# zahmedy/PyTorch-Distributed-Data-Parallel-DDP-Trainer

Hardware: AMD Instinct MI355X
Metric: images/sec MNIST SimpleCNN DDP at 1/2/4/8 MI355X; DDP scaling efficiency (higher is better)
Workload: dtype bf16; 1 GPU; model=SimpleCNN (520,586 params), global_batch=32, per_rank_batch=32, image=1x28x28, parallelism=dp1, engine=fused hipGraph, graph_steps=7, graph_head=0, fuse_level=3, level3=True, params_finite=True, bucket_allreduce=none, params_identical_across_ranks=True, ranks_seen=1, force_allreduce=False, inlaunch_allreduce=False

## Files before the change

### csrc/bindings.cpp

```cpp
#include <torch/extension.h>
#include <c10/hip/HIPStream.h>

#include <optional>

#include "kernels/conv_infer.h"
#include "kernels/launchers.h"
#include "runtime/runtime.h"

namespace py = pybind11;
using at::Tensor;
using namespace ddp_amd;

extern "C" const char ddp_amd_source_hash_str[];

namespace {

hipStream_t cur_stream() { return c10::hip::getCurrentHIPStream().stream(); }

void check_cuda(const Tensor& t, const char* name) {
  TORCH_CHECK(t.is_cuda(), name, " must be a GPU tensor");
  TORCH_CHECK(t.is_contiguous(), name, " must be contiguous");
}
void check(const Tensor& t, const char* name, at::ScalarType st) {
  check_cuda(t, name);
// ... 1292 lines not shown
             c.wgrad_rows = cfgd["wgrad_rows"].cast<int>();
             c.world = cfgd["world"].cast<int>(); c.rank = cfgd["rank"].cast<int>();
             c.lr = cfgd["lr"].cast<float>(); c.momentum = cfgd["momentum"].cast<float>();
             c.dampening = cfgd["dampening"].cast<float>();
             c.weight_decay = cfgd["weight_decay"].cast<float>();
             c.nesterov = cfgd["nesterov"].cast<bool>(); c.maximize = cfgd["maximize"].cast<bool>();
             c.force_allreduce = cfgd.contains("force_allreduce") ? cfgd["force_allreduce"].cast<bool>() : false;
             c.fuse_level = cfgd.contains("fuse_level") ? cfgd["fuse_level"].cast<int>() : 0;
             c.fuse_opt = cfgd.contains("fuse_opt") ? (int)cfgd["fuse_opt"].cast<bool>() : 1;
             c.store_a1 = cfgd.contains("store_a1") ? cfgd["store_a1"].cast<int>() : 0;
             c.f32 = cfgd.contains("f32") ? (int)cfgd["f32"].cast<bool>() : 0;
             c.fuse_reduce = cfgd.contains("fuse_reduce") ? cfgd["fuse_reduce"].cast<int>() : 1;
             c.wgrad_split = cfgd.contains("wgrad_split") ? cfgd["wgrad_split"].cast<int>() : 1;
             c.l3_fc_role = cfgd.contains("l3_fc_role") ? cfgd["l3_fc_role"].cast<int>() : 1;
             c.dist_mode = cfgd.contains("dist_mode") ? cfgd["dist_mode"].cast<int>() : 3;
             TORCH_CHECK(c.dist_mode >= 0 && c.dist_mode <= 4, "engine: dist_mode must be 0..4");
             TORCH_CHECK(c.l3_fc_role == 0 || c.l3_fc_role == 1, "engine: l3_fc_role must be 0 or 1");
             TORCH_CHECK(c.wgrad_split == 1 || c.wgrad_split == 2, "engine: wgrad_split must be 1 or 2");
             const int es = c.f32 ? 4 : 2;
             TORCH_CHECK(c.store_a1 >= 0 && c.store_a1 <= 2, "engine: store_a1 must be 0, 1 or 2");
             TORCH_CHECK(c.fuse_level == 0 || c.fuse_level == 1 || c.fuse_level == 3,
                         "engine: fuse_level must be 0, 1 or 3 (level 2 was removed in round 4)");
             TORCH_CHECK(conv3x3_fwd_lds(c.W, c.C1, c.pxt_fwd, c.fuse_level > 0, es) <= 160 * 1024 &&
                             conv3x3_wgrad_lds(c.W, c.C1, c.C2, c.wgrad_rows, c.fuse_level > 0, es) <= 160 * 1024 &&
                             conv3x3_dgrad_lds(c.W, c.C2, c.pxt_dgrad, true, es) <= 160 * 1024,
                         "engine: LDS budget exceeded for this tiling");
             auto T = [&](const char* k) { return t[k].cast<Tensor>(); };
             auto need = [&](const char* k, at::ScalarType st, long n) {
               Tensor x = T(k);
               check(x, k, st);
// ... 70 lines not shown
      .def("capture", &SimpleCNNEngine::capture)
      .def("replay", &SimpleCNNEngine::replay)
      .def("destroy_graph", &SimpleCNNEngine::destroy_graph)
      .def("synchronize", &SimpleCNNEngine::synchronize, py::call_guard<py::gil_scoped_release>())
      .def_property_readonly("last_fused_reduce", &SimpleCNNEngine::last_fused_reduce)
      .def_property_readonly("last_level3", &SimpleCNNEngine::last_level3)
      .def_property_readonly("last_fc_role", &SimpleCNNEngine::last_fc_role)
      .def_property_readonly("last_xar", &SimpleCNNEngine::last_xar)
      .def_property_readonly("last_pair", &SimpleCNNEngine::last_pair)
      .def_property_readonly("last_head", &SimpleCNNEngine::last_head)
      .def_property_readonly("graph_heads", &SimpleCNNEngine::graph_heads)
      .def("overlap_active", &SimpleCNNEngine::overlap_active)
      .def("level3_active", &SimpleCNNEngine::level3_active, py::arg("batch"))
      .def_property_readonly("sync_error", &SimpleCNNEngine::sync_error)
      .def("set_momentum_started", &SimpleCNNEngine::set_momentum_started)
      .def("set_xgmi", &SimpleCNNEngine::set_xgmi, py::arg("xgmi"), py::arg("channels"))
      .def_property_readonly("num_buckets", &SimpleCNNEngine::num_buckets)
      .def("bucket_stage", &SimpleCNNEngine::bucket_stage)
      .def_property_readonly("graph_steps", &SimpleCNNEngine::graph_steps)
      .def_property_readonly("stream", [](SimpleCNNEngine& e) { return (uint64_t)e.stream(); });
}
```

### csrc/kernels/conv3x3_fwd_body.inc.h

```cpp
  using P = Prec<T>;
  constexpr bool F32 = sizeof(T) == 4;
  static_assert(!DZ || (NOF == 10 && A1X), "level-3 dZ2 needs the fc epilogue and the conv1 recompute");
  static_assert(!MRG || (DZ && !F32), "the merged forward is the bf16 level-3 forward");
  constexpr int CE = P::CE;
  DDP_STAMP(STAMP_K_CONV_FWD, 0);
  DDP_GEOM_OVERRIDE();
  typedef __attribute__((address_space(1))) unsigned long long gran_t;
  constexpr int DZ_SW = (OCC == 2 || F32) ? XENT_MAX_BLK / 2 : XENT_MAX_BLK;
  unsigned dz_epoch = 1u;
  if constexpr (DZ) {
    const unsigned g = *dzo.gen + 1u;
    dz_epoch = g ? g : 1u;
  }
  constexpr int CH = 16 * NW * PXT, NT = NW * 64;
  const int lane = threadIdx.x & 63, wave = threadIdx.x >> 6;
  const int HW = H * W;
  const long Ptot = (long)B * HW;
  const int co0 = by * 64;
  const int KW = 9 * Cin, WS = KW + P::PAD, XS = Cin + P::PAD;
  const int XR = CH + 2 * W + 2;
  T* sW = reinterpret_cast<T*>(smem);
  T* sX = sW + 64 * WS;
  const long P0 = (long)bx * CH;
  const long Pbase = P0 - W - 1;

  const int wc = KW / CE;
// ... 9 lines not shown
  if (A1X) cg = conv1_group_load(c1.w, c1.b, wave & 3);
  stage2<(64 / NW) * (F32 ? 2 : 1), NT>(64 * wc,
             [&](int i) { const int r = i / wc, c = (i - r * wc) * CE; return ld16(Wt + (long)(co0 + r) * KW + c); },
             [&](int i, bf16x8 v) { const int r = i / wc, c = (i - r * wc) * CE; st16(sW + r * WS + c, v); },
             A1X ? 0 : XR * xc,
             [&](int i) {
               const int r = i / xc, c = (i - r * xc) * CE;
               const long Pq = Pbase + r;
               return (Pq >= 0 && Pq < Ptot) ? ld16(X + Pq * Cin + c) : zero8();
             },
             [&](int i, bf16x8 v) { const int r = i / xc, c = (i - r * xc) * CE; st16(sX + r * XS + c, v); });
  }
  if (A1X) {
    float* sxx = reinterpret_cast<float*>(sX + XR * XS);
    const int NXX = XR + 2 * W + 2;
    const int base = bi_base = c1.bi.base();
    for (int r = threadIdx.x; r < NXX; r += NT) {
      const long Pq = Pbase - W - 1 + r;
      float v = 0.f;
      if (Pq >= 0 && Pq < Ptot) {
        const int n = (int)(Pq / HW), rm = (int)(Pq - (long)n * HW);
        const int row = c1.bi.row(n, base);
        const unsigned char u = c1.x[(long)row * HW + rm];
        v = (float)u / 255.0f;
        if (c1.xb_out && Pq >= P0 && Pq < P0 + CH) {
          c1.xb_out[Pq] = u;
          if (rm == 0) c1.yb_out[n] = c1.labels[row];
        }
      }
      sxx[r] = v;
    }
    if constexpr (MRG) {
      DDP_STAMP(STAMP_K_HEAD, 4);
      wait_count<MRG_SLEEP>(mg.conv_done, mg.nblk1, mg.err, MRG_ERR);
      DDP_STAMP(STAMP_K_HEAD, 5);
      cg = conv1_group_load_sc1(c1.w, c1.b, wave & 3);
      const __amdgpu_buffer_rsrc_t rw =
          __builtin_amdgcn_make_buffer_rsrc(const_cast<T*>(Wt), (short)0, 0x7fffffff, 0x00020000);
      stage2<64 / NW, NT>(64 * wc,
          [&](int i) { const int r = i / wc, c = (i - r * wc) * CE; return ld16_sc1(rw, (int)(((co0 + r) * KW + c) * sizeof(T))); },
          [&](int i, bf16x8 v) { const int r = i / wc, c = (i - r * wc) * CE; st16(sW + r * WS + c, v); },
          0, [&](int) { return zero8(); }, [&](int, bf16x8) {});
// ... 245 lines not shown
          const int co = co0 + 16 * t + 4 * (lane >> 4);
          if (!valid[pt]) continue;
          if constexpr (F32) st_wt(reinterpret_cast<float4*>(Y + Pp[pt] * Cout + co), a2q[pt][t]);
          else st_wt(reinterpret_cast<uint2*>(Y + Pp[pt] * Cout + co), a2pk[pt][t]);
        }
    };
    DDP_STAMP(STAMP_K_FWD_DZ, 0);
    store_a2();
    if (wave == 0) {
      const int slot = lane >= NOF ? 1 : 0, o = lane - slot * NOF;
      const bool act = lane < 2 * NOF && slot < nimg;
      int label = 0;
      float fcb = 0.f;
      if (lane < 2 * NOF) {
        const int im = img0 + slot;
        if (im < B) label = c1.labels[c1.bi.row(im, bi_base)];
        fcb = MRG ? __hip_atomic_load(dzo.fc_bias + o, __ATOMIC_RELAXED, __HIP_MEMORY_SCOPE_AGENT) : dzo.fc_bias[o];
      }
      const int im = img0 + (act ? slot : 0);
      const int nblk = (im * HWi + HWi - 1) / CH - im * HWi / CH + 1;
      const gran_t* gr = (const gran_t*)dzo.gran;
      const unsigned long long t0 = __builtin_amdgcn_s_memrealtime();
      bool dead = false;
      float a = 0.f;
      DDP_STAMP(STAMP_K_FWD_DZ, 1);
      auto sweep = [&](auto j0c) {
        constexpr int J0 = decltype(j0c)::value;
        unsigned long long g[DZ_SW];
#pragma unroll
        for (int k = 0; k < DZ_SW; ++k) g[k] = 0;
        const bool none = J0 > 0 && !__any(act && nblk > J0);
// ... 86 lines not shown
```

### csrc/kernels/fc_bwd_body.h

```cpp
#pragma once
#include "kernels/common.h"
#include "kernels/launchers.h"

namespace ddp_amd {

constexpr int FCB_RB = 8;

template <int CPL>
struct ColF {
  float v[CPL];
};
template <int CPL>
__device__ __forceinline__ ColF<CPL> ldc(const bf16_t* p) {
  ColF<CPL> r;
  if constexpr (CPL == 2) {
    const unsigned u = *reinterpret_cast<const unsigned*>(p);
    r.v[0] = __builtin_bit_cast(float, u << 16);
    r.v[1] = __builtin_bit_cast(float, u & 0xffff0000u);
  } else {
    const uint2 u = *reinterpret_cast<const uint2*>(p);
    r.v[0] = __builtin_bit_cast(float, u.x << 16);
    r.v[1] = __builtin_bit_cast(float, u.x & 0xffff0000u);
    r.v[2] = __builtin_bit_cast(float, u.y << 16);
    r.v[3] = __builtin_bit_cast(float, u.y & 0xffff0000u);
// ... 55 lines not shown
    }
  }
  if ((XENT || ex.loss_rows) && ex.loss_out) {
    const float* lr = XENT ? s_loss : ex.loss_rows;
    const int at = ex.step_ctr ? *ex.step_ctr : 0;
    float acc = 0.f;
    for (int b0 = 0; b0 < B; b0 += 64) {
      const float v = b0 + lane < B ? lr[b0 + lane] : 0.f;
      const int nb = B - b0 < 64 ? B - b0 : 64;
      for (int k = 0; k < nb; ++k)
        acc += __builtin_bit_cast(float, __builtin_amdgcn_readlane(__builtin_bit_cast(int, v), k));
    }
    if (lane == 63) {
      ex.loss_out[at] = acc / (float)B;
      if (last && ex.step_inc) *ex.step_inc = at + 1;
    }
  }
  if (last || !ex.last_ctr) {
    if (ex.zero_i32)
      for (int i = lane; i < ex.n_zero; i += 64) ex.zero_i32[(long)i * ex.zero_stride] = 0;
    if (ex.gen_inc && lane == 0) {
      const unsigned g = *ex.gen_inc + 1u;
      *ex.gen_inc = g == 0xffffffffu ? 0u : g;
    }
  }
}

constexpr int FCDW_LD = 12;
template <int MAXB, typename T>
__device__ __forceinline__ void fc_dw_wave_chunk(const float* s_dl, const T* __restrict__ X,
// ... 273 lines not shown
```

### csrc/kernels/launchers.h

```cpp
#pragma once
#include <hip/hip_runtime.h>
#include <stdint.h>

#include "kernels/types.h"

namespace ddp_amd {

void stamps_set(void* buf);

void conv1_fwd(const void* x, bool x_is_u8, BatchIdx bi, const float* w, const float* b, bf16_t* y,
               int B, int H, int W, int Cout, hipStream_t s);
void conv1_fwd(const void* x, bool x_is_u8, BatchIdx bi, const float* w, const float* b, float* y,
               int B, int H, int W, int Cout, hipStream_t s);
int conv1_wgrad_blocks(int B, int H, int W, int chunk);
void conv1_wgrad(const void* x, bool x_is_u8, BatchIdx bi, const bf16_t* dy, const bf16_t* yact,
                 float* slab, int B, int H, int W, int Cout, int chunk, hipStream_t s);
void conv1_wgrad(const void* x, bool x_is_u8, BatchIdx bi, const float* dy, const float* yact,
                 float* slab, int B, int H, int W, int Cout, int chunk, hipStream_t s);

constexpr int FWD_DZ_CNT_STRIDE = 64;
struct FwdDz {
  bf16_t* dz2 = nullptr;
  float* dz2_f32 = nullptr;
  unsigned long long* gran = nullptr;
// ... 146 lines not shown
  const int* labels32 = nullptr;
  BatchIdx bi{};
  float gscale = 1.f;
  SgdArgs sgd{};
  float* p_w = nullptr;
  float* m_w = nullptr;
  bf16_t* sh_plain = nullptr;
  bf16_t* sh_frag = nullptr;
  float* sh_frag32 = nullptr;
  int frag_HW = 0, frag_C = 0;
  int sys_store = 0;
  int* last_ctr = nullptr;
  float* p_b = nullptr;
  float* m_b = nullptr;
  int* step_inc = nullptr;
  unsigned* gen_inc = nullptr;
  int* zero_i32 = nullptr;
  int n_zero = 0, zero_stride = 1;
  int last_n = 0;
};
struct BwdFc {
  const void* a2 = nullptr;
  const float* dl = nullptr;
  float* dW = nullptr;
  float scale = 1.f;
  long K = 0;
  int nconv = 0, fc0 = 0, nfc = 0;
  FcBwdExtras ex{};
};
size_t fc_bwd_lds(int B, int NO, bool xent, long npart = 0);
void noop(int blocks, int* sink, hipStream_t s);
void fc_bwd(const float* dL, const bf16_t* X, const bf16_t* Wf, bf16_t* dX, float* dW, float scale,
            int B, long K, int NO, bool mask, hipStream_t s, const FcBwdExtras& ex = FcBwdExtras());
void fc_bwd(const float* dL, const float* X, const float* Wf, float* dX, float* dW, float scale,
            int B, long K, int NO, bool mask, hipStream_t s, const FcBwdExtras& ex = FcBwdExtras());

void xent(const float* part, int G, const float* bias, int C, int B, const long long* labels64,
          const int* labels32, BatchIdx bi, float* logits_out, float* dlogits, float* loss_out,
          float* dbias, float gscale, float dbias_scale, hipStream_t s);

bool xent_wave_rows(const float* logits, int C, int B, const long long* labels, float* dlogits,
                    float* loss_out, float gscale, hipStream_t s);

void xent_rows(const float* part, int HW, int CH, const float* bias, int NO, int B,
               const int* labels32, BatchIdx bi, float* dlogits, float* loss_rows, float gscale,
               hipStream_t s);

enum { SHADOW_BF16 = 1, SHADOW_BF16_TAPT = 2, SHADOW_BF16_FCFRAG = 3, SHADOW_BF16_PAD4 = 4,
       SHADOW_F32_TAPT = 5, SHADOW_F32_FCFRAG = 6 };
constexpr int MAX_SHADOWS = 4;
// ... 119 lines not shown
```

### csrc/kernels/types.h

```cpp
#pragma once
#include <hip/hip_runtime.h>
#include <stdint.h>

namespace ddp_amd {

typedef unsigned short bf16_t;

struct BatchIdx {
  const int* idx;
  const int* step_ctr;
  int batch_stride;
  int offset;
  int n_idx = 0x7fffffff;
  int n_rows = 0x7fffffff;
  __device__ __forceinline__ int base() const {
    return step_ctr ? (*step_ctr) * batch_stride : offset;
  }
  __device__ __forceinline__ int row(int b, int base_) const {
    if (!idx) {
      const int r = base_ + b;
      return r < 0 ? 0 : (r >= n_rows ? n_rows - 1 : r);
    }
    int i = base_ + b;
    i = i < 0 ? 0 : (i >= n_idx ? n_idx - 1 : i);
    int r = idx[i];
    return r < 0 ? 0 : (r >= n_rows ? n_rows - 1 : r);
  }
};

struct C1Src {
  const unsigned char* x = nullptr;
  BatchIdx bi{};
  const float* w = nullptr;
  const float* b = nullptr;
  unsigned char* xb_out = nullptr;
  int* yb_out = nullptr;
  const int* labels = nullptr;
  bf16_t* a1_out = nullptr;
  int* zero_i32 = nullptr;
  int zero_per_block = 0;
  int zero_total = 0x7fffffff;
};

struct SgdArgs {
  float lr, momentum, dampening, weight_decay;
  int nesterov, maximize, first_step, update;
};

struct SchedState {
  int t, ticket;
  float lr_used;
};
// ... 22 lines not shown
```

### csrc/runtime/engine.cpp

```cpp
#include <algorithm>
#include <cstdio>
#include <cstdlib>
#include <cstring>
#include <type_traits>

#include "runtime/runtime.h"

namespace ddp_amd {

SimpleCNNEngine::SimpleCNNEngine(const EngineConfig& cfg, const EngineBuffers& buf,
                                 std::shared_ptr<Comm> comm, std::vector<EngineBucket> buckets)
    : cfg_(cfg), b_(buf), comm_(std::move(comm)), buckets_(std::move(buckets)) {
  if (cfg_.C1 != 32) throw std::runtime_error("engine: fused conv1 wgrad needs C1 == 32");
  if (cfg_.C2 % 64 != 0) throw std::runtime_error("engine: C2 must be a multiple of 64");
  if ((cfg_.H * cfg_.W) % 16 != 0) throw std::runtime_error("engine: H*W must be a multiple of 16");
  if (cfg_.NO != 10) throw std::runtime_error("engine: the fused fc epilogue is built for 10 classes");
  if (cfg_.f32 && (cfg_.fuse_level < 1 || cfg_.store_a1 != 0))
    throw std::runtime_error("engine: fp32 mode needs fuse_level >= 1 (level 1 or 3) and store_a1 0");
  if (cfg_.f32 && !(b_.a2_f32 && b_.dz2_f32 && b_.w2t_f32 && b_.wfc_frag32))
    throw std::runtime_error("engine: fp32 mode needs the a2 / dz2 / w2t / wfc_frag32 fp32 buffers");
  const long conv0 = std::min(std::min(b_.off_w2, b_.off_b2), std::min(b_.off_w1, b_.off_b1));
  const long fc_hi = std::max(b_.off_wfc + (long)cfg_.NO * cfg_.H * cfg_.W * cfg_.C2, b_.off_bfc + cfg_.NO);
  if (fc_hi > conv0) throw std::runtime_error("engine: fc gradients must precede the conv gradients");
  long prev_end = 0;
// ... 13 lines not shown
  l3_fits_.assign(cfg_.max_batch + 1, -1);
  if (b_.sync_err) {
    DDP_HIP_CHECK(hipHostMalloc(reinterpret_cast<void**>(&err_host_), sizeof(int),
                                hipHostMallocCoherent | hipHostMallocMapped));
    *err_host_ = 0;
    int* dev = nullptr;
    DDP_HIP_CHECK(hipHostGetDevicePointer(reinterpret_cast<void**>(&dev), err_host_, 0));
    b_.sync_err = dev;
  }
  if (cfg_.fuse_level >= 3 && b_.sync_flags && b_.sync_err) {
    const size_t ng = 2 * (size_t)cfg_.NO * (size_t)conv3x3_dgrad_blocks(cfg_.max_batch, cfg_.H, cfg_.W, 1);
    DDP_HIP_CHECK(hipMalloc(reinterpret_cast<void**>(&gran_), ng * sizeof(unsigned long long)));
    DDP_HIP_CHECK(hipMalloc(reinterpret_cast<void**>(&gen_), 256));
    DDP_HIP_CHECK(hipMemset(gran_, 0, ng * sizeof(unsigned long long)));
    DDP_HIP_CHECK(hipMemset(gen_, 0, 256));
    DDP_HIP_CHECK(hipStreamSynchronize(nullptr));
  }
}

SimpleCNNEngine::~SimpleCNNEngine() {
  if (process_exiting()) return;
  if (cs_) hipStreamSynchronize(cs_);
  destroy_graph();
  for (hipEvent_t e : {e_b0_, e_b1_, e_d0_, e_d1_, e_fwd_, e_fc_}) hipEventDestroy(e);
  for (XarArgs& e : xar_cache_) hipFree(const_cast<XgmiArgs*>(e.dev));
  if (err_host_) hipHostFree(err_host_);
  if (gran_) hipFree(gran_);
  if (gen_) hipFree(gen_);
}

void SimpleCNNEngine::destroy_graph() {
  if (graph_exec_) hipGraphExecDestroy(graph_exec_);
  if (graph_) hipGraphDestroy(graph_);
  graph_exec_ = nullptr;
  graph_ = nullptr;
  graph_steps_ = 0;
}

void SimpleCNNEngine::synchronize() {
  DDP_HIP_CHECK(hipStreamSynchronize(cs_));
  if (const int e = sync_error()) {
    throw std::runtime_error(std::string("engine: an in-launch hand-off wait timed out (") +
                             (e == RED_ERR ? "fused slab reduction" : e == XAR_ERR ? "in-launch all-reduce"
// ... 69 lines not shown
  if constexpr (std::is_same<T, float>::value)
    return {b.params + b.off_w2, b.w2t_f32, b.a2_f32, b.dz2_f32, b.wfc_frag32, b.params + b.off_wfc, nullptr, sh};
  else
    return {b.w2_bf16, b.w2t_bf16, b.a2, b.dz2, b.wfc_frag, b.wfc_bf16, b.a1, sh};
}

}

void SimpleCNNEngine::launch_step(int B, int stride, bool first_momentum_step, unsigned parts) {
  if (cfg_.f32)
    launch_step_t<float>(B, stride, first_momentum_step, parts);
  else
    launch_step_t<bf16_t>(B, stride, first_momentum_step, parts);
}

C1Src SimpleCNNEngine::make_c1src(int B, int stride, const StepPlan& pl) const {
  C1Src c1;
  c1.x = b_.images;
  c1.bi = BatchIdx{b_.idx, b_.step_ctr, stride, 0};
  c1.bi.n_idx = b_.n_idx;
  c1.bi.n_rows = b_.n_rows;
  c1.w = b_.params + b_.off_w1;
  c1.b = b_.params + b_.off_b1;
  c1.xb_out = b_.xb;
  c1.yb_out = b_.yb;
  c1.labels = b_.labels;
  if (cfg_.store_a1) c1.a1_out = b_.a1;
  if (pl.fred || pl.l3 || pl.pair_mode) {
    const int nfwd = conv3x3_dgrad_blocks(B, cfg_.H, cfg_.W, cfg_.pxt_fwd);
    const int nsync = SYNC_RED_INTS + ((pl.l3 || pl.pair_mode) ? L3_FC_INTS : 0);
    c1.zero_i32 = b_.sync_flags;
    c1.zero_per_block = (nsync + nfwd - 1) / nfwd;
    c1.zero_total = nsync;
  }
  return c1;
}

FwdDz SimpleCNNEngine::make_fwd_dz(int B) const {
  FwdDz dz;
  if (cfg_.f32) dz.dz2_f32 = b_.dz2_f32;
  else dz.dz2 = b_.dz2;
  dz.gran = gran_;
  dz.gen = gen_;
  dz.fc_bias = b_.params + b_.off_bfc;
  dz.gscale = 1.f / (float)B;
  dz.err = b_.sync_err;
  dz.dl_out = b_.dlogits;
  dz.loss_rows = b_.loss_rows;
  return dz;
}

FcBwdExtras SimpleCNNEngine::make_fc_extras(int B, const StepPlan& pl, const SgdArgs& sa) const {
  float* P = b_.params;
  float* M = b_.momentum;
  FcBwdExtras ex;
  ex.dbias = b_.grads + b_.off_bfc;
  ex.dbias_scale = 1.f / (float)cfg_.world;
  ex.loss_out = b_.loss_hist;
  ex.step_ctr = b_.step_ctr;
  ex.loss_rows = (pl.l3 || !pl.f1) ? b_.loss_rows : nullptr;
  if (pl.f1) {
    ex.part = pl.l3 ? nullptr : b_.fc_part;
    ex.HW = cfg_.H * cfg_.W;
    ex.CH = 64 * cfg_.pxt_fwd;
    ex.fc_bias = P + b_.off_bfc;
    ex.labels32 = b_.yb;
    ex.bi = BatchIdx{nullptr, nullptr, 0, 0};
// ... 15 lines not shown
    ex.frag_C = cfg_.C2;
  }
  if (pl.l3) {
    ex.gen_inc = gen_;
    if (pl.ov) {
      ex.zero_i32 = b_.sync_flags + L3_HEAD_OFF;
      ex.n_zero = 2;
      ex.zero_stride = FWD_DZ_CNT_STRIDE;
    }
  }
  if (pl.fc_role) {
    if (pl.fopt) {
      ex.p_b = P + b_.off_bfc;
      ex.m_b = M ? M + b_.off_bfc : nullptr;
    }
    if (pl.fopt || pl.ov) ex.step_inc = b_.step_ctr;
  }
  return ex;
}

SlabSet SimpleCNNEngine::make_slabs(int B, const StepPlan& pl, const SgdArgs& sa) const {
  const int C1 = cfg_.C1, C2 = cfg_.C2, NO = cfg_.NO;
  const long n_w2 = (long)C2 * 9 * C1, w2row = n_w2 + C2;
  const float inv_ws = 1.f / (float)cfg_.world;
  float* G = b_.grads;
  SlabSet ss{};
  const int wblk = conv3x3_wgrad_blocks(B, cfg_.H, cfg_.wgrad_rows);
  ss.s[0] = SlabSeg{b_.w2slab, w2row, 0, n_w2, wblk, G + b_.off_w2, inv_ws};
  ss.s[1] = SlabSeg{b_.w2slab, w2row, n_w2, (long)C2, wblk, G + b_.off_b2, inv_ws};
  const int dblk = conv3x3_dgrad_blocks(B, cfg_.H, cfg_.W, cfg_.pxt_dgrad);
  ss.s[2] = SlabSeg{b_.w1slab, 320, 0, (long)C1 * 9, dblk, G + b_.off_w1, inv_ws};
// ... 63 lines not shown
  const StepPlan pl = plan(B);
  if ((parts & (PART_HEAD | PART_AR)) && !pl.ov && parts != PART_ALL)
    throw std::runtime_error("engine: a split step needs the dist_mode 4 chain");
  if (BF16 && !pl.l3 && plain_stale_) {
    refresh_shadows();
    plain_stale_ = false;
  }
  const StepOperands<T> op = step_operands<T>(b_, shadow_set(!pl.l3));
  float* P = b_.params;
  float* G = b_.grads;
  float* M = b_.momentum;
  const float inv_ws = 1.f / (float)cfg_.world;
  const SgdArgs sa{cfg_.lr, cfg_.momentum, cfg_.dampening, cfg_.weight_decay, cfg_.nesterov,
                   cfg_.maximize, first_momentum_step ? 1 : 0, 1};

  const C1Src c1 = make_c1src(B, stride, pl);
  const FwdDz dzo = pl.l3 ? make_fwd_dz(B) : FwdDz{};
  bool head_used = false;
  if constexpr (BF16) {
    if (parts & PART_HEAD) {
      if (first_momentum_step) throw std::runtime_error("engine: the step head runs the steady-state SGD only");
      head_used = launch_step_head(B, sa, op.sh, c1, dzo);
    }
  }
  if ((parts & PART_FWD) || ((parts & PART_HEAD) && !head_used)) {
    if constexpr (BF16) {
      if (!pl.f1) conv1_fwd(b_.images, true, c1.bi, P + b_.off_w1, P + b_.off_b1, b_.a1, B, H, W, C1, cs_);
    }
    conv3x3_fwd(pl.f1 ? nullptr : op.a1, op.w2, P + b_.off_b2, op.a2, B, H, W, C1, C2, true, op.wfc_frag,
                b_.fc_part, NO, cfg_.pxt_fwd, cs_, pl.f1 ? &c1 : nullptr, pl.l3 ? &dzo : nullptr);
  }
  if (parts & (PART_FWD | PART_HEAD)) last_head_ = head_used;
  if (head_used && capturing_) graph_heads_ += 1;
  if (!(parts & (PART_BWD | PART_AR))) return;

  if constexpr (BF16) {
    if (!pl.f1)
      xent_rows(b_.fc_part, HW, 64 * cfg_.pxt_fwd, P + b_.off_bfc, NO, B, b_.labels, c1.bi, b_.dlogits,
                b_.loss_rows, 1.f / (float)B, cs_);
  }
  const FcBwdExtras ex = make_fc_extras(B, pl, sa);
  float* dWfc = pl.fopt ? nullptr : G + b_.off_wfc;
  const long K = (long)HW * C2;
  BwdFc fcr;
  std::function<void(hipStream_t)> fc_launch;
  if (pl.fc_role) {
    fcr.a2 = op.a2;
    fcr.dl = b_.dlogits;
    fcr.dW = dWfc;
    fcr.scale = inv_ws;
    fcr.K = K;
    fcr.ex = ex;
  } else {
    fc_launch = [&](hipStream_t s) {
      fc_bwd(b_.dlogits, op.a2, pl.l3 ? nullptr : op.wfc, pl.l3 ? nullptr : op.dz2, dWfc, inv_ws, B, K, NO,
             true, s, ex);
// ... 214 lines not shown
  }
}

void SimpleCNNEngine::step(int batch, int batch_stride) {
  const bool first = cfg_.momentum != 0.f && !momentum_started_;
  launch_step(batch, batch_stride, first);
  if (cfg_.momentum != 0.f) momentum_started_ = true;
  DDP_HIP_CHECK(hipGetLastError());
}

void SimpleCNNEngine::capture(int nsteps) {
  if (cfg_.momentum != 0.f && !momentum_started_)
    throw std::runtime_error("engine: run one eager step before capturing (momentum init)");
  destroy_graph();
  graph_heads_ = 0;
  capturing_ = true;
  DDP_HIP_CHECK(hipStreamBeginCapture(cs_, hipStreamCaptureModeRelaxed));
  try {
    if (overlap_active()) {
      for (int i = 0; i < nsteps; ++i)
        launch_step(cfg_.max_batch, cfg_.max_batch, false, (i == 0 ? PART_FWD : PART_HEAD) | PART_BWD);
      launch_step(cfg_.max_batch, cfg_.max_batch, false, PART_AR);
    } else {
      for (int i = 0; i < nsteps; ++i) launch_step(cfg_.max_batch, cfg_.max_batch, false);
    }
  } catch (...) {
    capturing_ = false;
    hipGraph_t g = nullptr;
    hipStreamEndCapture(cs_, &g);
    if (g) hipGraphDestroy(g);
    throw;
  }
  capturing_ = false;
  DDP_HIP_CHECK(hipStreamEndCapture(cs_, &graph_));
  DDP_HIP_CHECK(hipGraphInstantiate(&graph_exec_, graph_, nullptr, nullptr, 0));
  const char* up = std::getenv("DDP_AMD_GRAPH_UPLOAD");
  if (!(up && up[0] == '0')) {
    DDP_HIP_CHECK(hipGraphUpload(graph_exec_, cs_));
    DDP_HIP_CHECK(hipStreamSynchronize(cs_));
  }
  graph_steps_ = nsteps;
}

void SimpleCNNEngine::replay() {
  if (!graph_exec_) throw std::runtime_error("engine: no captured graph");
  DDP_HIP_CHECK(hipGraphLaunch(graph_exec_, cs_));
}

}
```

### csrc/runtime/runtime.h

```cpp
#pragma once
#include <hip/hip_runtime.h>
#include <rccl/rccl.h>

#include <functional>
#include <memory>
#include <stdexcept>
#include <string>
#include <vector>

#include "kernels/launchers.h"
#include "runtime/bucket_state.h"
#include "runtime/step_plan.h"

#define DDP_HIP_CHECK(expr)                                                              \
  do {                                                                                   \
    hipError_t _e = (expr);                                                              \
    if (_e != hipSuccess)                                                                \
      throw std::runtime_error(std::string("HIP error ") + hipGetErrorString(_e) + " at " + \
                               __FILE__ + ":" + std::to_string(__LINE__) + ": " #expr);  \
  } while (0)

#define DDP_NCCL_CHECK(expr)                                                             \
  do {                                                                                   \
    ncclResult_t _r = (expr);                                                            \
// ... 211 lines not shown
  bool has_graph() const { return graph_exec_ != nullptr; }
  int graph_steps() const { return graph_steps_; }
  void destroy_graph();
  hipStream_t stream() const { return cs_; }
  void synchronize();
  int sync_error() const { return err_host_ ? __atomic_load_n(err_host_, __ATOMIC_ACQUIRE) : 0; }
  bool level3_active(int batch) { return plan(batch).l3; }
  bool overlap_active() { return plan(cfg_.max_batch).ov && pair_plan_ok_ && cfg_.pxt_fwd == 1; }
  bool last_fused_reduce() const { return last_fused_reduce_; }
  bool last_level3() const { return last_level3_; }
  bool last_fc_role() const { return last_fc_role_; }
  bool last_xar() const { return last_xar_; }
  bool last_pair() const { return last_pair_; }
  bool last_head() const { return last_head_; }
  int graph_heads() const { return graph_heads_; }
  void set_momentum_started(bool v) { momentum_started_ = v; }
  void set_xgmi(std::shared_ptr<XgmiComm> x, std::vector<int> channels);
  int num_buckets() const { return (int)buckets_.size(); }
  int bucket_stage(int b) const { return stage_.at(b); }

 private:
  enum : unsigned { PART_FWD = 1, PART_BWD = 2, PART_AR = 4, PART_HEAD = 8, PART_ALL = 7 };
  void launch_step(int batch, int batch_stride, bool first_momentum_step, unsigned parts = PART_ALL);
  template <typename T>
  void launch_step_t(int batch, int batch_stride, bool first_momentum_step, unsigned parts);
  StepPlan plan(int batch);
  ShadowSet shadow_set(bool plain_fc) const;
  C1Src make_c1src(int B, int stride, const StepPlan& pl) const;
  FwdDz make_fwd_dz(int B) const;
  FcBwdExtras make_fc_extras(int B, const StepPlan& pl, const SgdArgs& sa) const;
  SlabSet make_slabs(int B, const StepPlan& pl, const SgdArgs& sa) const;
  bool launch_step_head(int B, const SgdArgs& sa, const ShadowSet& sh, const C1Src& c1, const FwdDz& dzo);
  void launch_buckets(int stage, bool use_x, const SgdArgs& sa, float* M, const ShadowSet& sh);
  void join_buckets();
  void enqueue_buckets(int stage, bool use_x, hipStream_t s, const SgdArgs& sa, float* M, const ShadowSet& sh);
  void schedule_backward(bool dist, bool fork, bool use_x, const std::function<void(hipStream_t)>& fc,
                         const std::function<void()>& conv, const SgdArgs& sa, float* M, const ShadowSet& sh);
  bool late_shadow_ok(long off, long n) const;
  bool make_xar(BwdXar& xa, const SgdArgs& sa, float* M, const ShadowSet& sh);
  bool sync_ok_for_xar() const;
  EngineConfig cfg_;
  EngineBuffers b_;
  std::shared_ptr<Comm> comm_;
  std::shared_ptr<XgmiComm> xgmi_;
  std::vector<EngineBucket> buckets_;
  std::vector<int> stage_;
  std::vector<int> xch_;
  int last_bucket_ = -1;
  bool stage_used_[2] = {false, false};
  hipStream_t cs_ = nullptr, ms_ = nullptr;
  hipEvent_t e_b0_, e_b1_, e_d0_, e_d1_, e_fwd_, e_fc_;
  std::vector<signed char> l3_fits_;
  hipGraph_t graph_ = nullptr;
  hipGraphExec_t graph_exec_ = nullptr;
// ... 7 lines not shown
  bool last_head_ = false;
  bool capturing_ = false;
  int graph_heads_ = 0;
  bool xar_plan_ok_ = false;
  bool pair_plan_ok_ = false;
  struct XarArgs {
    XgmiArgs host[2];
    const XgmiArgs* dev = nullptr;
  };
  std::vector<XarArgs> xar_cache_;
  hipStream_t xs_ = nullptr;
  bool plain_stale_ = false;
  int* err_host_ = nullptr;
  unsigned long long* gran_ = nullptr;
  unsigned* gen_ = nullptr;
};

}
```

### csrc/runtime/step_plan.h

```cpp
#pragma once

namespace ddp_amd {

struct EngineConfig {
  int max_batch, H, W, C1, C2, NO;
  int pxt_fwd, pxt_dgrad, wgrad_rows;
  int world, rank;
  float lr, momentum, dampening, weight_decay;
  int nesterov, maximize;
  int force_allreduce;
  int fuse_level = 0;
  int l3_fc_role = 1;
  int fuse_opt = 1;
  int store_a1 = 0;
  int f32 = 0;
  int fuse_reduce = 1;
  int wgrad_split = 1;
  int dist_mode = 3;
};

struct StepFacts {
  bool xgmi = false;
  int xgmi_world = 1;
  bool comm = false;
  int comm_world = 1;
  bool sync_flags = false, sync_err = false;
  bool l3_fits = false;
  bool fc_role_ok = false;
  bool xar_plan_ok = false;
};

struct StepPlan {
  bool use_x;
// ... 34 lines not shown
```

### pytorch-distributed-data-parallel-ddp-trainer_amd/engine/fused_step.py

```python
from __future__ import annotations

import dataclasses
import os
import math

import torch

from .. import native
from ..data.loader import DeviceMNIST
from ..data.sampler import ShardedSampler
from ..models.layers import flat_space
from ..ops.functional import wgrad_rows
from ..parallel.ddp import bucket_plan, bucket_ranges

from ..parallel.bucket_model import ONESHOT_MAX_ELEMS

BF16 = torch.bfloat16


@dataclasses.dataclass
class EngineOptions:
    graph_steps: int = 100
    use_graph: bool = True
    pxt_fwd: int | None = None
# ... 4 lines not shown
    bucket_plan: str = "model"
    force_allreduce: bool = False
    fuse_level: int = 3
    l3_fc_role: int = 1
    fuse_opt: bool = True
    fuse_reduce: int | None = None
    store_a1: int | None = None
    comm: str = "auto"
    epoch_order: bool = True
    dtype: str = "bf16"
    wgrad_split: int = 2
    dist_mode: int = 4
    xar_blocks: int = 96
    plan_world: int | None = None
    cost_fit: dict | None = None


def agree(store, key: str, rank: int, world: int, ok: bool) -> bool:
    if store is None or world <= 1:
        return bool(ok)
    store.set(f"{key}/{rank}", b"1" if ok else b"0")
    return all(store.get(f"{key}/{r}") == b"1" for r in range(world))



def gather_rank_sum(local: torch.Tensor, world: int) -> torch.Tensor:
    import torch.distributed as dist

    src = local.detach().float().contiguous()
    if world <= 1 or not dist.is_initialized():
# ... 133 lines not shown
                    else data.labels_i32),
            idx=torch.zeros(n_rank, dtype=torch.int32, device=dev),
        )
        nfl = 256 + 32 + 64 * 2
        self.t["sync_flags"] = torch.zeros(nfl, dtype=torch.int32, device=dev)
        self.t["sync_err"] = torch.zeros(1, dtype=torch.int32, device=dev)
        cfg = dict(max_batch=B, H=28, W=28, C1=32, C2=64, NO=10, pxt_fwd=self.opts.pxt_fwd,
                   pxt_dgrad=self.opts.pxt_dgrad, wgrad_rows=R, world=world_size, rank=rank,
                   lr=float(g["lr"]), momentum=float(g["momentum"]),
                   dampening=float(g["dampening"]), weight_decay=float(g["weight_decay"]),
                   nesterov=bool(g["nesterov"]), maximize=bool(g["maximize"]),
                   force_allreduce=bool(self.opts.force_allreduce),
                   fuse_level=self._fuse_level_ok(world_size), fuse_opt=bool(self.opts.fuse_opt),
                   store_a1=int(self.store_a1), f32=f32, fuse_reduce=self._fuse_reduce_ok(world_size),
                   epoch_order=bool(self.opts.epoch_order), wgrad_split=int(self.opts.wgrad_split),
                   l3_fc_role=int(self.opts.l3_fc_role), dist_mode=int(self.opts.dist_mode))
        self.dtype = "fp32" if f32 else "bf16"
        use_comm = world_size > 1 or self.opts.force_allreduce
        self.xgmi = None
        self.xgmi_plan = None
        self.allreduce_us = None
        xch = list(range(len(ranges)))
        if use_comm and self.opts.comm in ("auto", "tune", "xgmi", "xgmi1", "xgmi2"):
            from ..parallel.xgmi import channel_plan, create_xgmi, pick_data_plane

            lim = self.cost.oneshot_cap_elems()
            oneshot = tuple(b for b, (_, n) in enumerate(ranges) if n <= lim)
            from ..parallel.xgmi import ENGINE_GRID_CAP

            cap = int(self.opts.xar_blocks) if self.opts.dist_mode == 2 else ENGINE_GRID_CAP
            self.xgmi = create_xgmi(fs.grads, ranges, rank, world_size, oneshot=oneshot, grid_cap=cap)
# ... 56 lines not shown
            store = dist.distributed_c10d._get_default_store()
        t = self.t
        keys = ("params", "momentum", "step_ctr", "loss_hist")
        self.synchronize()
        torch.cuda.synchronize()
        snap = {k: t[k].clone() for k in keys}
        started = self.opt.momentum_buffer is not None and self.opt.steps > 0
        B = self.B

        def restore(e):
            with torch.cuda.stream(self.stream):
                for k in keys:
                    t[k].copy_(snap[k])
            torch.cuda.synchronize()
            e.set_momentum_started(started)
            e.refresh_shadows()
            torch.cuda.synchronize()

        head = bool(self.eng.overlap_active())
        if head:
            nsteps = max(nsteps, 3)

        def run(e, graph=False):
            self.start_epoch(0)
            restore(e)
            try:
                if graph:
                    left = nsteps
                    if self.opt.momentum_buffer is not None and not started:
                        e.step(B, B)
# ... 146 lines not shown
    def _log_downgrade(self, what: str):
        self.downgrades = getattr(self, "downgrades", []) + [what]
        if self.rank == 0:
            import sys

            print(f"[ddp_amd] engine: {what}", file=sys.stderr)

    def sync_from_torch(self):
        ev = torch.cuda.Event()
        ev.record(torch.cuda.current_stream())
        self.stream.wait_event(ev)

    def refresh(self):
        self.sync_from_torch()
        self.eng.refresh_shadows()

    def synchronize(self):
        self.eng.synchronize()
        self._check_xgmi("step")

    def _check_xgmi(self, where: str):
        if self.xgmi is not None:
            code = self.xgmi.error_flags()
            if code:
                from ..parallel.xgmi import describe_xgmi_error

                raise RuntimeError(f"xGMI all-reduce ({where}) on rank {self.rank}: "
                                   f"{describe_xgmi_error(code)}; results invalid")

    def _start_barrier(self):
# ... 58 lines not shown
                out.record_stream(torch.cuda.current_stream())
        return res

    def start_epoch(self, epoch: int):
        self.sampler.set_epoch(epoch)
        idx = self.sampler.indices().to(torch.int32)
        with torch.cuda.stream(self.stream):
            self.t["idx"].copy_(idx)
            if self.opts.epoch_order:
                n, HW = self.t["idx"].numel(), 28 * 28
                torch.index_select(self.data.images_u8.view(-1, HW), 0, self.t["idx"],
                                   out=self.t["images"].view(n, HW))
                torch.index_select(self.data.labels_i32, 0, self.t["idx"], out=self.t["labels"])
            self.t["step_ctr"].zero_()
            self.t["loss_hist"].zero_()

    def run_epoch(self, epoch: int, on_loss=None, log_every: int = 100, max_steps: int | None = None):
        self._start_barrier()
        self.sync_from_torch()
        self.start_epoch(epoch)
        n = len(self.sampler)
        B = self.B
        nfull, rem = divmod(n, B)
        if max_steps is not None and max_steps < nfull + (1 if rem else 0):
            nfull, rem = max_steps, 0
        done = 0
        pending = []
        if self.opt.momentum_buffer is not None and not self.opt.steps and nfull > 0:
            self.eng.step(B, B)
            done, self.opt.steps = 1, 1
# ... 43 lines not shown
            else:
                self._wrap_if_needed(1, n_full)
                self.eng.step(self.B, self.B)
                done += 1
        self.steps_done += done
        self.opt.steps += done - init
        return done

    _bench_started = False
    _bench_pos = 0

    def _wrap_if_needed(self, k, n_full):
        if self._bench_pos + k > n_full:
            with torch.cuda.stream(self.stream):
                self.t["step_ctr"].zero_()
            self._bench_pos = 0
        self._bench_pos += k

    def _event(self):
        ev = torch.cuda.Event()
        ev.record(self.stream)
        return ev

    def _drain(self, pending, on_loss, log_every, keep):
        while len(pending) > keep:
            first, last, ev = pending.pop(0)
            want = [b for b in range(first, last) if b % log_every == 0]
            if not want or on_loss is None:
                continue
            ev.synchronize()
# ... 4 lines not shown
```

Baseline: 1.007 million images/sec.

## Precompute next step's batch rows and labels in fc backward epilogue record

Adds a small device-side step record that the fc backward tail fills with the next step's gathered row indices, labels and generation counter. The level-3 forward reads rows, labels and the epoch from this record instead of chasing the index-then-label indirection and loading the generation counter. The aim is to cut dependent global loads from the forward's critical path. In exchange it adds a record buffer, an init kernel on epoch starts and wraps, and host-side validity tracking that must stay consistent with graph replays.

```diff
diff --git a/csrc/bindings.cpp b/csrc/bindings.cpp
--- a/csrc/bindings.cpp
+++ b/csrc/bindings.cpp
@@ -1330,6 +1330,7 @@
              c.wgrad_split = cfgd.contains("wgrad_split") ? cfgd["wgrad_split"].cast<int>() : 1;
              c.l3_fc_role = cfgd.contains("l3_fc_role") ? cfgd["l3_fc_role"].cast<int>() : 1;
              c.dist_mode = cfgd.contains("dist_mode") ? cfgd["dist_mode"].cast<int>() : 3;
+             c.step_record = cfgd.contains("step_record") ? (int)cfgd["step_record"].cast<bool>() : 1;
              TORCH_CHECK(c.dist_mode >= 0 && c.dist_mode <= 4, "engine: dist_mode must be 0..4");
              TORCH_CHECK(c.l3_fc_role == 0 || c.l3_fc_role == 1, "engine: l3_fc_role must be 0 or 1");
              TORCH_CHECK(c.wgrad_split == 1 || c.wgrad_split == 2, "engine: wgrad_split must be 1 or 2");
@@ -1430,6 +1431,23 @@
       .def("level3_active", &SimpleCNNEngine::level3_active, py::arg("batch"))
       .def_property_readonly("sync_error", &SimpleCNNEngine::sync_error)
       .def("set_momentum_started", &SimpleCNNEngine::set_momentum_started)
+      .def("record_init", &SimpleCNNEngine::record_init)
+      .def("record_active", &SimpleCNNEngine::record_active, py::arg("batch"))
+      .def_property_readonly("last_record", &SimpleCNNEngine::last_record)
+      .def("read_record", [](SimpleCNNEngine& e) -> py::object {
+             const std::vector<int> w = e.read_record();
+             if (w.empty()) return py::none();
+             const int n = w[2];
+             py::dict d;
+             d["gen"] = (unsigned)w[0];
+             d["base"] = w[1];
+             d["n"] = n;
+             d["stride"] = w[3];
+             TORCH_CHECK(n >= 0 && (size_t)step_rec_ints(n) <= w.size(), "engine: step record header out of range");
+             d["rows"] = std::vector<int>(w.begin() + STEP_REC_HDR, w.begin() + STEP_REC_HDR + n);
+             d["labels"] = std::vector<int>(w.begin() + STEP_REC_HDR + n, w.begin() + STEP_REC_HDR + 2 * n);
+             return d;
+           })
       .def("set_xgmi", &SimpleCNNEngine::set_xgmi, py::arg("xgmi"), py::arg("channels"))
       .def_property_readonly("num_buckets", &SimpleCNNEngine::num_buckets)
       .def("bucket_stage", &SimpleCNNEngine::bucket_stage)
diff --git a/csrc/kernels/conv3x3_fwd_body.inc.h b/csrc/kernels/conv3x3_fwd_body.inc.h
--- a/csrc/kernels/conv3x3_fwd_body.inc.h
+++ b/csrc/kernels/conv3x3_fwd_body.inc.h
@@ -8,8 +8,9 @@
   typedef __attribute__((address_space(1))) unsigned long long gran_t;
   constexpr int DZ_SW = (OCC == 2 || F32) ? XENT_MAX_BLK / 2 : XENT_MAX_BLK;
   unsigned dz_epoch = 1u;
+  const int* const rec = A1X ? c1.rec : nullptr;
   if constexpr (DZ) {
-    const unsigned g = *dzo.gen + 1u;
+    const unsigned g = (rec ? (unsigned)rec[0] : *dzo.gen) + 1u;
     dz_epoch = g ? g : 1u;
   }
   constexpr int CH = 16 * NW * PXT, NT = NW * 64;
@@ -49,18 +50,18 @@
   if (A1X) {
     float* sxx = reinterpret_cast<float*>(sX + XR * XS);
     const int NXX = XR + 2 * W + 2;
-    const int base = bi_base = c1.bi.base();
+    const int base = bi_base = rec ? 0 : c1.bi.base();
     for (int r = threadIdx.x; r < NXX; r += NT) {
       const long Pq = Pbase - W - 1 + r;
       float v = 0.f;
       if (Pq >= 0 && Pq < Ptot) {
         const int n = (int)(Pq / HW), rm = (int)(Pq - (long)n * HW);
-        const int row = c1.bi.row(n, base);
+        const int row = rec ? rec[STEP_REC_HDR + n] : c1.bi.row(n, base);
         const unsigned char u = c1.x[(long)row * HW + rm];
         v = (float)u / 255.0f;
         if (c1.xb_out && Pq >= P0 && Pq < P0 + CH) {
           c1.xb_out[Pq] = u;
-          if (rm == 0) c1.yb_out[n] = c1.labels[row];
+          if (rm == 0) c1.yb_out[n] = rec ? rec[STEP_REC_HDR + c1.rec_n + n] : c1.labels[row];
         }
       }
       sxx[r] = v;
@@ -336,7 +337,7 @@
       float fcb = 0.f;
       if (lane < 2 * NOF) {
         const int im = img0 + slot;
-        if (im < B) label = c1.labels[c1.bi.row(im, bi_base)];
+        if (im < B) label = rec ? rec[STEP_REC_HDR + c1.rec_n + im] : c1.labels[c1.bi.row(im, bi_base)];
         fcb = MRG ? __hip_atomic_load(dzo.fc_bias + o, __ATOMIC_RELAXED, __HIP_MEMORY_SCOPE_AGENT) : dzo.fc_bias[o];
       }
       const int im = img0 + (act ? slot : 0);
diff --git a/csrc/kernels/fc_bwd_body.h b/csrc/kernels/fc_bwd_body.h
--- a/csrc/kernels/fc_bwd_body.h
+++ b/csrc/kernels/fc_bwd_body.h
@@ -93,6 +93,14 @@
     if (lane == 63) {
       ex.loss_out[at] = acc / (float)B;
       if (last && ex.step_inc) *ex.step_inc = at + 1;
+    }
+    if (last && ex.step_inc && ex.rec.rec) {
+      unsigned g = 0;
+      if (ex.gen_inc) {
+        g = *ex.gen_inc + 1u;
+        g = g == 0xffffffffu ? 0u : g;
+      }
+      step_rec_refresh(ex.rec, at + 1, g, lane);
     }
   }
   if (last || !ex.last_ctr) {
diff --git a/csrc/kernels/launchers.h b/csrc/kernels/launchers.h
--- a/csrc/kernels/launchers.h
+++ b/csrc/kernels/launchers.h
@@ -184,6 +184,7 @@
   float* p_b = nullptr;
   float* m_b = nullptr;
   int* step_inc = nullptr;
+  StepRec rec{};
   unsigned* gen_inc = nullptr;
   int* zero_i32 = nullptr;
   int n_zero = 0, zero_stride = 1;
@@ -204,6 +205,8 @@
             int B, long K, int NO, bool mask, hipStream_t s, const FcBwdExtras& ex = FcBwdExtras());
 void fc_bwd(const float* dL, const float* X, const float* Wf, float* dX, float* dW, float scale,
             int B, long K, int NO, bool mask, hipStream_t s, const FcBwdExtras& ex = FcBwdExtras());
+
+void step_rec_init(const StepRec& r, const int* step_ctr, const unsigned* gen, hipStream_t s);
 
 void xent(const float* part, int G, const float* bias, int C, int B, const long long* labels64,
           const int* labels32, BatchIdx bi, float* logits_out, float* dlogits, float* loss_out,
diff --git a/csrc/kernels/step_rec.hip b/csrc/kernels/step_rec.hip
--- /dev/null
+++ b/csrc/kernels/step_rec.hip
@@ -0,0 +1,15 @@
+#include "kernels/launchers.h"
+
+namespace ddp_amd {
+
+__global__ __launch_bounds__(64) void step_rec_init_kernel(StepRec r, const int* __restrict__ step_ctr,
+                                                           const unsigned* __restrict__ gen) {
+  step_rec_refresh(r, step_ctr ? *step_ctr : 0, gen ? *gen : 0u, (int)threadIdx.x);
+}
+
+void step_rec_init(const StepRec& r, const int* step_ctr, const unsigned* gen, hipStream_t s) {
+  if (!r.rec || r.n <= 0 || r.n > STEP_REC_MAXN) return;
+  hipLaunchKernelGGL(step_rec_init_kernel, dim3(1), dim3(64), 0, s, r, step_ctr, gen);
+}
+
+}
diff --git a/csrc/kernels/types.h b/csrc/kernels/types.h
--- a/csrc/kernels/types.h
+++ b/csrc/kernels/types.h
@@ -28,6 +28,31 @@
   }
 };
 
+constexpr int STEP_REC_HDR = 4;
+constexpr int STEP_REC_MAXN = 64;
+__host__ __device__ inline int step_rec_ints(int n) { return STEP_REC_HDR + 2 * n; }
+struct StepRec {
+  int* rec = nullptr;
+  const int* labels = nullptr;
+  BatchIdx bi{};
+  int n = 0;
+};
+__device__ __forceinline__ void step_rec_refresh(const StepRec& r, int step, unsigned gen, int lane) {
+  const int base = step * r.bi.batch_stride;
+  if (lane < r.n) {
+    const int row = r.bi.row(lane, base);
+    const int lab = r.labels[row];
+    r.rec[STEP_REC_HDR + lane] = row;
+    r.rec[STEP_REC_HDR + r.n + lane] = lab;
+  }
+  if (lane == 0) {
+    r.rec[0] = (int)gen;
+    r.rec[1] = base;
+    r.rec[2] = r.n;
+    r.rec[3] = r.bi.batch_stride;
+  }
+}
+
 struct C1Src {
   const unsigned char* x = nullptr;
   BatchIdx bi{};
@@ -36,6 +61,8 @@
   unsigned char* xb_out = nullptr;
   int* yb_out = nullptr;
   const int* labels = nullptr;
+  const int* rec = nullptr;
+  int rec_n = 0;
   bf16_t* a1_out = nullptr;
   int* zero_i32 = nullptr;
   int zero_per_block = 0;
diff --git a/csrc/runtime/engine.cpp b/csrc/runtime/engine.cpp
--- a/csrc/runtime/engine.cpp
+++ b/csrc/runtime/engine.cpp
@@ -51,6 +51,11 @@
     DDP_HIP_CHECK(hipMalloc(reinterpret_cast<void**>(&gen_), 256));
     DDP_HIP_CHECK(hipMemset(gran_, 0, ng * sizeof(unsigned long long)));
     DDP_HIP_CHECK(hipMemset(gen_, 0, 256));
+    if (cfg_.step_record && cfg_.max_batch <= STEP_REC_MAXN && b_.labels && b_.step_ctr) {
+      const size_t nb = std::max<size_t>(512, sizeof(int) * (size_t)step_rec_ints(cfg_.max_batch));
+      DDP_HIP_CHECK(hipMalloc(reinterpret_cast<void**>(&rec_), nb));
+      DDP_HIP_CHECK(hipMemset(rec_, 0, nb));
+    }
     DDP_HIP_CHECK(hipStreamSynchronize(nullptr));
   }
 }
@@ -64,6 +69,7 @@
   if (err_host_) hipHostFree(err_host_);
   if (gran_) hipFree(gran_);
   if (gen_) hipFree(gen_);
+  if (rec_) hipFree(rec_);
 }
 
 void SimpleCNNEngine::destroy_graph() {
@@ -163,7 +169,7 @@
     launch_step_t<bf16_t>(B, stride, first_momentum_step, parts);
 }
 
-C1Src SimpleCNNEngine::make_c1src(int B, int stride, const StepPlan& pl) const {
+C1Src SimpleCNNEngine::make_c1src(int B, int stride, const StepPlan& pl, bool use_rec) const {
   C1Src c1;
   c1.x = b_.images;
   c1.bi = BatchIdx{b_.idx, b_.step_ctr, stride, 0};
@@ -174,6 +180,10 @@
   c1.xb_out = b_.xb;
   c1.yb_out = b_.yb;
   c1.labels = b_.labels;
+  if (use_rec) {
+    c1.rec = rec_;
+    c1.rec_n = cfg_.max_batch;
+  }
   if (cfg_.store_a1) c1.a1_out = b_.a1;
   if (pl.fred || pl.l3 || pl.pair_mode) {
     const int nfwd = conv3x3_dgrad_blocks(B, cfg_.H, cfg_.W, cfg_.pxt_fwd);
@@ -183,6 +193,34 @@
     c1.zero_total = nsync;
   }
   return c1;
+}
+
+StepRec SimpleCNNEngine::make_rec(int stride) const {
+  StepRec r;
+  r.rec = rec_;
+  r.labels = b_.labels;
+  r.bi = BatchIdx{b_.idx, nullptr, stride, 0};
+  r.bi.n_idx = b_.n_idx;
+  r.bi.n_rows = b_.n_rows;
+  r.n = cfg_.max_batch;
+  return r;
+}
+
+void SimpleCNNEngine::record_init() {
+  if (!rec_) return;
+  if (capturing_) throw std::runtime_error("engine: record_init during a graph capture");
+  step_rec_init(make_rec(cfg_.max_batch), b_.step_ctr, gen_, cs_);
+  DDP_HIP_CHECK(hipGetLastError());
+  rec_valid_ = true;
+}
+
+std::vector<int> SimpleCNNEngine::read_record() {
+  std::vector<int> out;
+  if (!rec_) return out;
+  out.resize((size_t)step_rec_ints(cfg_.max_batch));
+  DDP_HIP_CHECK(hipStreamSynchronize(cs_));
+  DDP_HIP_CHECK(hipMemcpy(out.data(), rec_, out.size() * sizeof(int), hipMemcpyDeviceToHost));
+  return out;
 }
 
 FwdDz SimpleCNNEngine::make_fwd_dz(int B) const {
@@ -199,7 +237,7 @@
   return dz;
 }
 
-FcBwdExtras SimpleCNNEngine::make_fc_extras(int B, const StepPlan& pl, const SgdArgs& sa) const {
+FcBwdExtras SimpleCNNEngine::make_fc_extras(int B, const StepPlan& pl, const SgdArgs& sa, const StepRec& rec) const {
   float* P = b_.params;
   float* M = b_.momentum;
   FcBwdExtras ex;
@@ -245,7 +283,10 @@
       ex.p_b = P + b_.off_bfc;
       ex.m_b = M ? M + b_.off_bfc : nullptr;
     }
-    if (pl.fopt || pl.ov) ex.step_inc = b_.step_ctr;
+    if (pl.fopt || pl.ov) {
+      ex.step_inc = b_.step_ctr;
+      ex.rec = rec;
+    }
   }
   return ex;
 }
@@ -339,7 +380,12 @@
   const SgdArgs sa{cfg_.lr, cfg_.momentum, cfg_.dampening, cfg_.weight_decay, cfg_.nesterov,
                    cfg_.maximize, first_momentum_step ? 1 : 0, 1};
 
-  const C1Src c1 = make_c1src(B, stride, pl);
+  const bool keep_rec = record_chain(pl) && stride == cfg_.max_batch;
+  if (keep_rec && (parts & (PART_FWD | PART_HEAD))) {
+    if (capturing_) graph_rec_ = true;
+    else if (!rec_valid_) record_init();
+  }
+  const C1Src c1 = make_c1src(B, stride, pl, keep_rec);
   const FwdDz dzo = pl.l3 ? make_fwd_dz(B) : FwdDz{};
   bool head_used = false;
   if constexpr (BF16) {
@@ -355,7 +401,10 @@
     conv3x3_fwd(pl.f1 ? nullptr : op.a1, op.w2, P + b_.off_b2, op.a2, B, H, W, C1, C2, true, op.wfc_frag,
                 b_.fc_part, NO, cfg_.pxt_fwd, cs_, pl.f1 ? &c1 : nullptr, pl.l3 ? &dzo : nullptr);
   }
-  if (parts & (PART_FWD | PART_HEAD)) last_head_ = head_used;
+  if (parts & (PART_FWD | PART_HEAD)) {
+    last_head_ = head_used;
+    last_record_ = keep_rec;
+  }
   if (head_used && capturing_) graph_heads_ += 1;
   if (!(parts & (PART_BWD | PART_AR))) return;
 
@@ -364,7 +413,8 @@
       xent_rows(b_.fc_part, HW, 64 * cfg_.pxt_fwd, P + b_.off_bfc, NO, B, b_.labels, c1.bi, b_.dlogits,
                 b_.loss_rows, 1.f / (float)B, cs_);
   }
-  const FcBwdExtras ex = make_fc_extras(B, pl, sa);
+  const FcBwdExtras ex = make_fc_extras(B, pl, sa, keep_rec ? make_rec(stride) : StepRec{});
+  if ((parts & PART_BWD) && !capturing_) rec_valid_ = keep_rec;
   float* dWfc = pl.fopt ? nullptr : G + b_.off_wfc;
   const long K = (long)HW * C2;
   BwdFc fcr;
@@ -609,6 +659,7 @@
     throw std::runtime_error("engine: run one eager step before capturing (momentum init)");
   destroy_graph();
   graph_heads_ = 0;
+  graph_rec_ = false;
   capturing_ = true;
   DDP_HIP_CHECK(hipStreamBeginCapture(cs_, hipStreamCaptureModeRelaxed));
   try {
@@ -639,7 +690,9 @@
 
 void SimpleCNNEngine::replay() {
   if (!graph_exec_) throw std::runtime_error("engine: no captured graph");
+  if (graph_rec_ && !rec_valid_) record_init();
   DDP_HIP_CHECK(hipGraphLaunch(graph_exec_, cs_));
-}
-
-}
+  rec_valid_ = graph_rec_;
+}
+
+}
diff --git a/csrc/runtime/runtime.h b/csrc/runtime/runtime.h
--- a/csrc/runtime/runtime.h
+++ b/csrc/runtime/runtime.h
@@ -249,6 +249,10 @@
   bool last_pair() const { return last_pair_; }
   bool last_head() const { return last_head_; }
   int graph_heads() const { return graph_heads_; }
+  void record_init();
+  bool record_active(int batch) { return record_chain(plan(batch)); }
+  bool last_record() const { return last_record_; }
+  std::vector<int> read_record();
   void set_momentum_started(bool v) { momentum_started_ = v; }
   void set_xgmi(std::shared_ptr<XgmiComm> x, std::vector<int> channels);
   int num_buckets() const { return (int)buckets_.size(); }
@@ -261,9 +265,9 @@
   void launch_step_t(int batch, int batch_stride, bool first_momentum_step, unsigned parts);
   StepPlan plan(int batch);
   ShadowSet shadow_set(bool plain_fc) const;
-  C1Src make_c1src(int B, int stride, const StepPlan& pl) const;
+  C1Src make_c1src(int B, int stride, const StepPlan& pl, bool use_rec) const;
   FwdDz make_fwd_dz(int B) const;
-  FcBwdExtras make_fc_extras(int B, const StepPlan& pl, const SgdArgs& sa) const;
+  FcBwdExtras make_fc_extras(int B, const StepPlan& pl, const SgdArgs& sa, const StepRec& rec) const;
   SlabSet make_slabs(int B, const StepPlan& pl, const SgdArgs& sa) const;
   bool launch_step_head(int B, const SgdArgs& sa, const ShadowSet& sh, const C1Src& c1, const FwdDz& dzo);
   void launch_buckets(int stage, bool use_x, const SgdArgs& sa, float* M, const ShadowSet& sh);
@@ -273,6 +277,10 @@
                          const std::function<void()>& conv, const SgdArgs& sa, float* M, const ShadowSet& sh);
   bool late_shadow_ok(long off, long n) const;
   bool make_xar(BwdXar& xa, const SgdArgs& sa, float* M, const ShadowSet& sh);
+  bool record_chain(const StepPlan& pl) const {
+    return rec_ && pl.l3 && pl.fc_role && (pl.fopt || (pl.ov && pair_plan_ok_));
+  }
+  StepRec make_rec(int stride) const;
   bool sync_ok_for_xar() const;
   EngineConfig cfg_;
   EngineBuffers b_;
@@ -310,6 +318,10 @@
   int* err_host_ = nullptr;
   unsigned long long* gran_ = nullptr;
   unsigned* gen_ = nullptr;
+  int* rec_ = nullptr;
+  bool rec_valid_ = false;
+  bool graph_rec_ = false;
+  bool last_record_ = false;
 };
 
 }
diff --git a/csrc/runtime/step_plan.h b/csrc/runtime/step_plan.h
--- a/csrc/runtime/step_plan.h
+++ b/csrc/runtime/step_plan.h
@@ -17,6 +17,7 @@
   int fuse_reduce = 1;
   int wgrad_split = 1;
   int dist_mode = 3;
+  int step_record = 1;
 };
 
 struct StepFacts {
diff --git a/pytorch-distributed-data-parallel-ddp-trainer_amd/engine/fused_step.py b/pytorch-distributed-data-parallel-ddp-trainer_amd/engine/fused_step.py
--- a/pytorch-distributed-data-parallel-ddp-trainer_amd/engine/fused_step.py
+++ b/pytorch-distributed-data-parallel-ddp-trainer_amd/engine/fused_step.py
@@ -42,6 +42,7 @@
     xar_blocks: int = 96
     plan_world: int | None = None
     cost_fit: dict | None = None
+    step_record: bool = True
 
 
 def agree(store, key: str, rank: int, world: int, ok: bool) -> bool:
@@ -205,7 +206,8 @@
                    fuse_level=self._fuse_level_ok(world_size), fuse_opt=bool(self.opts.fuse_opt),
                    store_a1=int(self.store_a1), f32=f32, fuse_reduce=self._fuse_reduce_ok(world_size),
                    epoch_order=bool(self.opts.epoch_order), wgrad_split=int(self.opts.wgrad_split),
-                   l3_fc_role=int(self.opts.l3_fc_role), dist_mode=int(self.opts.dist_mode))
+                   l3_fc_role=int(self.opts.l3_fc_role), dist_mode=int(self.opts.dist_mode),
+                   step_record=bool(self.opts.step_record))
         self.dtype = "fp32" if f32 else "bf16"
         use_comm = world_size > 1 or self.opts.force_allreduce
         self.xgmi = None
@@ -292,6 +294,7 @@
                     t[k].copy_(snap[k])
             torch.cuda.synchronize()
             e.set_momentum_started(started)
+            e.record_init()
             e.refresh_shadows()
             torch.cuda.synchronize()
 
@@ -468,6 +471,7 @@
     def refresh(self):
         self.sync_from_torch()
         self.eng.refresh_shadows()
+        self.eng.record_init()
 
     def synchronize(self):
         self.eng.synchronize()
@@ -556,6 +560,7 @@
                 torch.index_select(self.data.labels_i32, 0, self.t["idx"], out=self.t["labels"])
             self.t["step_ctr"].zero_()
             self.t["loss_hist"].zero_()
+            self.eng.record_init()
 
     def run_epoch(self, epoch: int, on_loss=None, log_every: int = 100, max_steps: int | None = None):
         self._start_barrier()
@@ -629,6 +634,7 @@
         if self._bench_pos + k > n_full:
             with torch.cuda.stream(self.stream):
                 self.t["step_ctr"].zero_()
+                self.eng.record_init()
             self._bench_pos = 0
         self._bench_pos += k
 
```

Result: no change. 1.008 million images/sec (median of 2 runs) (+0.1%).
